# delldu/TransMVSNet

Measured on AMD Instinct MI355X. Metric: depth maps/sec @ DTU 864x1152 N=5 (48/32/8 hyp); Abs depth L1 vs ref, higher is better.
Workload: dtype f32; 1 GPU; DTU 864x1152, N=5 views, cascade 48/32/8, B=1, hot path from FeatureNet outputs (FMT+pathway+stage glue+cost volume+CostRegNet+softmax/WTA); global_batch=1, parallelism=replica1, launch=hip_graph replay

## Files before the change

### transmvsnet_amd/csrc/common.h

```cpp
#pragma once

#include <hip/hip_runtime.h>
#include <stdint.h>

#include "../../include/transmvs.h"

#define TMVS_CHECK_LAUNCH()                                   \
  do {                                                        \
    hipError_t _e = hipGetLastError();                        \
    if (_e != hipSuccess) return TMVS_ERR_HIP;                \
  } while (0)

namespace tmvs {

__device__ __forceinline__ float relu(float x) { return x > 0.f ? x : 0.f; }

typedef float floatx4_t __attribute__((ext_vector_type(4)));

struct LinAxis {
  int i0, i1;
  float l0, l1;
};
__device__ __forceinline__ LinAxis lin_axis(int dst, int in_size, int out_size) {
  const float scale = (float)in_size / (float)out_size;
  float src = scale * ((float)dst + 0.5f) - 0.5f;
  src = src < 0.f ? 0.f : src;
  LinAxis a;
  a.i0 = min((int)floorf(src), in_size - 1);
  a.i1 = a.i0 + (a.i0 < in_size - 1 ? 1 : 0);
  const float l = fminf(fmaxf(src - (float)a.i0, 0.f), 1.f);
  a.l1 = l;
  a.l0 = 1.f - l;
  return a;
}
__device__ __forceinline__ LinAxis lin_axis_x2(int dst, int in_size) {
  float src = 0.5f * ((float)dst + 0.5f) - 0.5f;
  src = src < 0.f ? 0.f : src;
  LinAxis a;
  a.i0 = (int)src;
  a.i0 = a.i0 < in_size - 1 ? a.i0 : in_size - 1;
  a.i1 = a.i0 + (a.i0 < in_size - 1 ? 1 : 0);
  a.l1 = src - (float)a.i0;
  a.l0 = 1.f - a.l1;
  return a;
}

__device__ __forceinline__ bool xcd_range_tap(int ntaps, int nblk, int& rb, int& k) {
  const int per = 8 * ntaps;
  const int grp = blockIdx.x / per, within = blockIdx.x % per;
  k = within / 8;
  rb = grp * 8 + within % 8;
  return rb < nblk;
}
static inline dim3 xcd_range_tap_grid(int ntaps, int nblk) { return dim3((unsigned)((nblk + 7) / 8 * 8 * ntaps)); }

__device__ __forceinline__ void chunk_row_coords(long v, int H, int W, int& b, int& y, int& x) {
  const long vl = v & ~63L;
  const unsigned lo = __builtin_amdgcn_readfirstlane((unsigned)vl);
  const unsigned hi = __builtin_amdgcn_readfirstlane((unsigned)((unsigned long)vl >> 32));
  const long vb = (long)(((unsigned long)hi << 32) | lo);
  const long t = vb / W;
  x = (int)(vb - t * W) + (int)(v - vb);
  y = (int)(t % H);
  b = (int)(t / H);
  while (x >= W) {
    x -= W;
    if (++y == H) {
      y = 0;
      ++b;
    }
  }
}

__device__ __forceinline__ void chunk_row_coords3(long v, int D, int H, int W, int& b, int& z, int& y, int& x) {
  const long vl = v & ~63L;
  const unsigned lo = __builtin_amdgcn_readfirstlane((unsigned)vl);
  const unsigned hi = __builtin_amdgcn_readfirstlane((unsigned)((unsigned long)vl >> 32));
  const long vb = (long)(((unsigned long)hi << 32) | lo);
  long t = vb / W;
  x = (int)(vb - t * W) + (int)(v - vb);
  y = (int)(t % H);
  t /= H;
  z = (int)(t % D);
  b = (int)(t / D);
  while (x >= W) {
    x -= W;
    if (++y == H) {
      y = 0;
      if (++z == D) {
        z = 0;
        ++b;
      }
    }
  }
}

// ... 85 lines not shown
```

### transmvsnet_amd/csrc/fmt.hip

```cpp
#include "fmt_common.h"

namespace tmvs {

__global__ __launch_bounds__(256) void fmt_embed_kernel(const float* __restrict__ feat, long view_stride,
                                                        const float* __restrict__ pe, int pe_h, int pe_w, int H, int W,
                                                        int nv, float* __restrict__ tokens) {
  __shared__ float tile[64][kD + 1];
  const int HW = H * W;
  const int p0 = blockIdx.x * 64;
  const int px = threadIdx.x & 63, c0 = threadIdx.x >> 6;
  const int p = p0 + px;
  const bool in = p < HW;
  const int y = in ? p / W : 0, x = in ? p - y * W : 0;
  float pv[kD / 4];
#pragma unroll
  for (int k = 0; k < kD / 4; ++k) pv[k] = in ? pe[((size_t)(c0 + 4 * k) * pe_h + y) * pe_w + x] : 0.f;
  const int tp = threadIdx.x >> 3, q = threadIdx.x & 7;
  float t[kD / 4];
  auto load = [&](int v) {
    const float* f = feat + (size_t)v * view_stride;
#pragma unroll
    for (int k = 0; k < kD / 4; ++k) t[k] = in ? f[(size_t)(c0 + 4 * k) * HW + p] : 0.f;
  };
  load(0);
#pragma unroll 1
  for (int v = 0; v < nv; ++v) {
    __syncthreads();
#pragma unroll
    for (int k = 0; k < kD / 4; ++k) tile[px][c0 + 4 * k] = t[k] + pv[k];
    __syncthreads();
    if (v + 1 < nv) load(v + 1);
#pragma unroll
    for (int h = 0; h < 2; ++h) {
      const int r = tp + 32 * h;
      if (p0 + r < HW)
        *reinterpret_cast<float4*>(tokens + ((size_t)v * HW + p0 + r) * kD + 4 * q) =
            make_float4(tile[r][4 * q], tile[r][4 * q + 1], tile[r][4 * q + 2], tile[r][4 * q + 3]);
    }
  }
}

__device__ __forceinline__ int kfeat(int s, int g) { return 16 * (s >> 2) + 4 * g + (s & 3); }

template <int OUT, int IN, bool TRANS>
__device__ __forceinline__ void stage_afrag(const float* __restrict__ W, float* __restrict__ lds) {
  constexpr int N = OUT * IN;
  for (int idx = threadIdx.x; idx < N; idx += blockDim.x) {
    const int j = idx & 3, l = (idx >> 2) & 63, rest = idx >> 8;
    const int s4 = rest % (IN / 16), mb = rest / (IN / 16);
    const int s = 4 * s4 + j;
    const int o = 16 * mb + (l & 15), i = kfeat(s, l >> 4);
    lds[idx] = TRANS ? W[i * OUT + o] : W[o * IN + i];
  }
}

template <int OUT, int IN>
__device__ __forceinline__ void mfma_linear_lds(const float* __restrict__ fl, const floatx4_t (&in)[IN / 16],
                                                floatx4_t (&acc)[OUT / 16], int lane) {
#pragma unroll
  for (int mb = 0; mb < OUT / 16; ++mb) acc[mb] = floatx4_t{0.f, 0.f, 0.f, 0.f};
#pragma unroll
  for (int s4 = 0; s4 < IN / 16; ++s4) {
    float4 a4[OUT / 16];
#pragma unroll
    for (int mb = 0; mb < OUT / 16; ++mb) a4[mb] = ld4(fl + ((mb * (IN / 16) + s4) * 64 + lane) * 4);
#pragma unroll
    for (int j = 0; j < 4; ++j)
#pragma unroll
      for (int mb = 0; mb < OUT / 16; ++mb)
        acc[mb] = __builtin_amdgcn_mfma_f32_16x16x4f32(j == 0 ? a4[mb].x : j == 1 ? a4[mb].y : j == 2 ? a4[mb].z : a4[mb].w,
                                                       in[s4][j], acc[mb], 0, 0, 0);
  }
}

__device__ __forceinline__ int wave_index() { return __builtin_amdgcn_readfirstlane(threadIdx.x >> 6); }
__device__ __forceinline__ int first_tile(int wv, int tpw) { return (blockIdx.x * 4 + wv) * tpw; }
__device__ __forceinline__ int opaque_zero() {
  int salt = 0;
  asm volatile("" : "+s"(salt));
  return salt;
}
template <typename T>
__device__ __forceinline__ T* row(T* base, int t, int n) { return base + (size_t)(t < n ? t : n - 1) * kD; }
__device__ __forceinline__ void ld4(const float* p, float (&a)[4]) {
  const float4 t = ld4(p);
  a[0] = t.x, a[1] = t.y, a[2] = t.z, a[3] = t.w;
}

__device__ __forceinline__ float token_sum(float v) {
  v += __shfl_xor(v, 16, 64);
  v += __shfl_xor(v, 32, 64);
  return v;
}

__device__ __forceinline__ void layer_norm_frag(floatx4_t (&x)[2], const float* __restrict__ g,
                                                const float* __restrict__ b, int lane) {
  float s = 0.f;
#pragma unroll
  for (int mb = 0; mb < 2; ++mb)
#pragma unroll
    for (int r = 0; r < 4; ++r) s += x[mb][r];
  const float mean = token_sum(s) / (float)kD;
  float v = 0.f;
#pragma unroll
  for (int mb = 0; mb < 2; ++mb)
#pragma unroll
    for (int r = 0; r < 4; ++r) {
      const float d = x[mb][r] - mean;
      v = fmaf(d, d, v);
    }
  const float rstd = 1.f / sqrtf(token_sum(v) / (float)kD + kLnEps);
  const float bias = -rstd * mean;
#pragma unroll
  for (int mb = 0; mb < 2; ++mb) {
    float gg[4], bb[4];
    ld4(g + 16 * mb + 4 * (lane >> 4), gg);
    ld4(b + 16 * mb + 4 * (lane >> 4), bb);
#pragma unroll
    for (int r = 0; r < 4; ++r) x[mb][r] = fmaf(fmaf(x[mb][r], rstd, bias), gg[r], bb[r]);
  }
}

__device__ __forceinline__ void load_token_frag(const float* __restrict__ row, floatx4_t (&x)[2], int lane) {
#pragma unroll
  for (int mb = 0; mb < 2; ++mb) {
    const float4 t = ld4(row + 16 * mb + 4 * (lane >> 4));
    x[mb] = floatx4_t{t.x, t.y, t.z, t.w};
  }
}

constexpr int kKvTilesPerWave = 8;

template <int OFF>
__device__ __forceinline__ float xor_add(float x) {
  return x + __int_as_float(xor_lane_dpp<OFF>(__float_as_int(x)));
}
__device__ __forceinline__ float xor_sum16(float x) { return xor_add<8>(xor_add<4>(xor_add<2>(xor_add<1>(x)))); }

__global__ __launch_bounds__(256) void fmt_kv_partial_kernel(const float* __restrict__ src, int S,
                                                              const float* __restrict__ w,
                                                              float* __restrict__ partial, int tpw) {
  __shared__ float red[4][kKV];
  __shared__ __attribute__((aligned(16))) float frag[2 * 32 * 32];
  const int v = blockIdx.y;
  const int lane = threadIdx.x & 63, wv = wave_index();
  const int g = lane >> 4;
  stage_afrag<32, 32, true>(w + TMVS_ENC_WK, frag);
  stage_afrag<32, 32, true>(w + TMVS_ENC_WV, frag + 1024);
  float bk[2][4], bv[2][4];
#pragma unroll
  for (int mb = 0; mb < 2; ++mb)
#pragma unroll
    for (int r = 0; r < 4; ++r) {
      bk[mb][r] = w[TMVS_ENC_BK + 16 * mb + 4 * g + r];
      bv[mb][r] = w[TMVS_ENC_BV + 16 * mb + 4 * g + r];
    }
  float kv[2][16], ks[2][4];
#pragma unroll
  for (int mb = 0; mb < 2; ++mb) {
// ... 2 lines not shown
#pragma unroll
    for (int i = 0; i < 4; ++i) ks[mb][i] = 0.f;
  }
  __syncthreads();
  const float* sv = src + (size_t)v * S * kD;
  const int tile0 = first_tile(wv, tpw);
  floatx4_t xa[2], xb[2];
  if (tile0 * 16 < S) load_token_frag(row(sv, tile0 * 16 + (lane & 15), S), xa, lane);
  auto tile = [&](int it, floatx4_t (&cur)[2], floatx4_t (&nxt)[2]) {
    const float* fr = frag + opaque_zero();
    const int t = (tile0 + it) * 16 + (lane & 15);
    const bool ok = t < S;
    const floatx4_t xin[2] = {cur[0], cur[1]};
    floatx4_t kk[2], vv[2];
    load_token_frag(row(sv, t + 16, S), nxt, lane);
    mfma_linear_lds<32, 32>(fr, xin, kk, lane);
    mfma_linear_lds<32, 32>(fr + 1024, xin, vv, lane);
#pragma unroll
    for (int mb = 0; mb < 2; ++mb) {
      float kh[4], vh[4];
#pragma unroll
      for (int r = 0; r < 4; ++r) {
        kh[r] = ok ? elu1(kk[mb][r] + bk[mb][r]) : 0.f;
        vh[r] = ok ? vv[mb][r] + bv[mb][r] : 0.f;
      }
#pragma unroll
      for (int m = 0; m < 4; ++m)
#pragma unroll
        for (int d = 0; d < 4; ++d) kv[mb][m * 4 + d] = fmaf(kh[d], vh[m], kv[mb][m * 4 + d]);
#pragma unroll
      for (int d = 0; d < 4; ++d) ks[mb][d] += kh[d];
    }
  };
#pragma unroll 1
  for (int it = 0; it < tpw; ++it) {
    if ((tile0 + it) * 16 >= S) break;
    tile(it, xa, xb);
    xa[0] = xb[0];
    xa[1] = xb[1];
  }
#pragma unroll
  for (int mb = 0; mb < 2; ++mb) {
#pragma unroll
    for (int i = 0; i < 16; ++i) kv[mb][i] = xor_sum16(kv[mb][i]);
#pragma unroll
    for (int i = 0; i < 4; ++i) ks[mb][i] = xor_sum16(ks[mb][i]);
  }
  if ((lane & 15) == 0) {
#pragma unroll
    for (int mb = 0; mb < 2; ++mb) {
      const int h = 4 * mb + g;
#pragma unroll
      for (int i = 0; i < 16; ++i) red[wv][kv_at(h, i >> 2, i & 3)] = kv[mb][i];
#pragma unroll
      for (int i = 0; i < 4; ++i) red[wv][ksum_at(h, i)] = ks[mb][i];
    }
  }
  __syncthreads();
  if (threadIdx.x < kKV) {
    const int i = threadIdx.x;
    partial[((size_t)v * gridDim.x + blockIdx.x) * kKV + i] = (red[0][i] + red[1][i]) + (red[2][i] + red[3][i]);
  }
}

__global__ __launch_bounds__(1024) void fmt_kv_combine_kernel(const float* __restrict__ partial, int nblk,
                                                              float* __restrict__ kv) {
  __shared__ float red[32][32];
  const int v = blockIdx.x;
  const int e = blockIdx.y * 32 + (threadIdx.x & 31);
  const int g = threadIdx.x >> 5;
  float s = 0.f;
#pragma unroll 4
  for (int b = g; b < nblk; b += 32) s += partial[((size_t)v * nblk + b) * kKV + e];
  red[g][threadIdx.x & 31] = s;
  __syncthreads();
  if (g == 0) {
    float t = red[0][threadIdx.x];
#pragma unroll
    for (int k = 1; k < 32; ++k) t += red[k][threadIdx.x];
    kv[(size_t)v * kKV + e] = t;
  }
}

__global__ __launch_bounds__(256) void fmt_apply_kernel(float* __restrict__ x, int L, const float* __restrict__ kvg,
                                                        long kv_stride, const float* __restrict__ w, int tpw) {
  __shared__ __attribute__((aligned(16))) float kvs[kKV];
  constexpr int kVB2 = 128, kVLN = 160;
  __shared__ __attribute__((aligned(16))) float vec[288];
  const int v = blockIdx.y;
  const int lane = threadIdx.x & 63, wv = wave_index();
  const int g = lane >> 4;
  if (threadIdx.x < kKV) kvs[threadIdx.x] = kvg[(size_t)v * kv_stride + threadIdx.x];
  for (int i = threadIdx.x; i < 288; i += blockDim.x)
    vec[i] = i < 32 ? w[TMVS_ENC_BQ + i] : i < 64 ? w[TMVS_ENC_BO + i - 32] : i < 128 ? w[TMVS_ENC_B1 + i - 64]
                                                                                      : w[TMVS_ENC_B2 + i - kVB2];
  __shared__ __attribute__((aligned(16))) float frag[32 * 32 * 2 + 64 * 32 * 2];
  stage_afrag<32, 32, false>(w + TMVS_ENC_WQ, frag);
  stage_afrag<32, 32, false>(w + TMVS_ENC_WO, frag + 1024);
  stage_afrag<64, 32, false>(w + TMVS_ENC_W1, frag + 2048);
  stage_afrag<32, 64, true>(w + TMVS_ENC_W2T, frag + 4096);
  __syncthreads();
  float* xv = x + (size_t)v * L * kD;
  const int tile0 = first_tile(wv, tpw);
  floatx4_t xa[2], xb[2];
  load_token_frag(row(xv, tile0 * 16 + (lane & 15), L), xa, lane);
  auto tile = [&](int it, floatx4_t (&cur)[2], floatx4_t (&nxt)[2]) {
    const int salt = opaque_zero();
    const float* fr = frag + salt;
    const float* vb = vec + salt;
    const int t = (tile0 + it) * 16 + (lane & 15);
    const bool ok = t < L;
    float* out = row(xv, t, L);
    floatx4_t xs[2] = {cur[0], cur[1]};
    load_token_frag(row(xv, t + 16, L), nxt, lane);
    floatx4_t q[2], msg[2];
    mfma_linear_lds<32, 32>(fr, xs, q, lane);
#pragma unroll
    for (int mb = 0; mb < 2; ++mb) {
      const int h = 4 * mb + g;
      float bq[4], ksum[4], kvm[4][4];
      ld4(vb + 4 * h, bq);
      ld4(kvs + ksum_at(h, 0), ksum);
#pragma unroll
      for (int m = 0; m < 4; ++m) ld4(kvs + kv_at(h, m, 0), kvm[m]);
      float qe[4];
#pragma unroll
      for (int d = 0; d < 4; ++d) qe[d] = elu1(q[mb][d] + bq[d]);
      float den = 0.f;
#pragma unroll
      for (int d = 0; d < 4; ++d) den = fmaf(qe[d], ksum[d], den);
      const float z = 1.f / (den + kAttnEps);
#pragma unroll
      for (int m = 0; m < 4; ++m) {
        float num = 0.f;
#pragma unroll
        for (int d = 0; d < 4; ++d) num = fmaf(qe[d], kvm[m][d], num);
        msg[mb][m] = num * z;
      }
    }
    floatx4_t a[2];
    mfma_linear_lds<32, 32>(fr + 1024, msg, a, lane);
#pragma unroll
    for (int mb = 0; mb < 2; ++mb) {
      float bo[4];
      ld4(vb + 32 + 16 * mb + 4 * g, bo);
#pragma unroll
      for (int r = 0; r < 4; ++r) xs[mb][r] = xs[mb][r] + (a[mb][r] + bo[r]);
    }
    layer_norm_frag(xs, vb + kVLN, vb + kVLN + kD, lane);
    floatx4_t hdn[4], ff[2];
    mfma_linear_lds<64, 32>(fr + 2048, xs, hdn, lane);
#pragma unroll
    for (int mb = 0; mb < 4; ++mb) {
      float b1[4];
      ld4(vb + 64 + 16 * mb + 4 * g, b1);
#pragma unroll
      for (int r = 0; r < 4; ++r) hdn[mb][r] = relu(hdn[mb][r] + b1[r]);
    }
    mfma_linear_lds<32, 64>(fr + 4096, hdn, ff, lane);
#pragma unroll
    for (int mb = 0; mb < 2; ++mb) {
      float b2[4];
      ld4(vb + kVB2 + 16 * mb + 4 * g, b2);
#pragma unroll
      for (int r = 0; r < 4; ++r) xs[mb][r] = xs[mb][r] + (ff[mb][r] + b2[r]);
    }
    layer_norm_frag(xs, vb + kVLN + 2 * kD, vb + kVLN + 3 * kD, lane);
    if (ok) {
#pragma unroll
      for (int mb = 0; mb < 2; ++mb)
        *reinterpret_cast<float4*>(out + 16 * mb + 4 * g) = make_float4(xs[mb][0], xs[mb][1], xs[mb][2], xs[mb][3]);
    }
  };
#pragma unroll 1
  for (int it = 0; it < tpw; it += 2) {
    if ((tile0 + it) * 16 >= L) break;
    tile(it, xa, xb);
    if (it + 1 >= tpw || (tile0 + it + 1) * 16 >= L) break;
    tile(it + 1, xb, xa);
  }
}

template <typename K>
static long block_slots(K kernel) {
  int dev = 0, cus = 0, per = 0;
  (void)hipGetDevice(&dev);
  (void)hipDeviceGetAttribute(&cus, hipDeviceAttributeMultiprocessorCount, dev);
  if (hipOccupancyMaxActiveBlocksPerMultiprocessor(&per, kernel, 256, 0) != hipSuccess || per <= 0) per = 4;
  return (long)(cus > 0 ? cus : 256) * per;
}
static int wave_slots_apply() {
  static long slots = 0;
  if (!slots) slots = 4 * block_slots(fmt_apply_kernel);
  return (int)slots;
}

static int kv_tiles_per_wave(int nv, int S) {
  const int tiles = (S + 15) / 16;
  int tpw = kKvTilesPerWave;
  while (tpw > 2 && (long)nv * ((tiles + tpw - 1) / tpw) < 2048) tpw >>= 1;
  return tpw;
}
static int kv_nblk(int nv, int S) {
  const int per = 16 * 4 * kv_tiles_per_wave(nv, S);
  return (S + per - 1) / per;
}
static int apply_tiles_per_wave(int nv, int L) {
  const long tiles = (long)nv * ((L + 15) / 16);
  return (int)std::max<long>(1, (tiles + wave_slots_apply() - 1) / wave_slots_apply());
}
static int apply_nblk(int L, int tpw) { return (L + 16 * 4 * tpw - 1) / (16 * 4 * tpw); }

}

using namespace tmvs;

extern "C" int tmvs_fmt_embed(const float* feat, long feat_view_stride, const float* pe, int pe_h, int pe_w, int nv,
                              int channels, int height, int width, float* tokens, void* stream) {
  if (!feat || !pe || !tokens || nv <= 0 || height <= 0 || width <= 0) return TMVS_ERR_ARG;
  if (channels != kD || height > pe_h || width > pe_w) return TMVS_ERR_SHAPE;
  const int HW = height * width;
  hipLaunchKernelGGL(fmt_embed_kernel, dim3((HW + 63) / 64), dim3(256), 0, (hipStream_t)stream, feat,
                     feat_view_stride, pe, pe_h, pe_w, height, width, nv, tokens);
  TMVS_CHECK_LAUNCH();
  return TMVS_OK;
}

extern "C" size_t tmvs_fmt_kv_grouped_workspace(int nv, int group_nv, int s_tokens) {
  if (nv <= 0 || group_nv <= 0 || s_tokens <= 0) return 0;
  return (size_t)nv * kv_nblk(group_nv, s_tokens) * kKV * sizeof(float);
}

extern "C" size_t tmvs_fmt_kv_workspace(int nv, int s_tokens) { return tmvs_fmt_kv_grouped_workspace(nv, nv, s_tokens); }

extern "C" int tmvs_fmt_kv_grouped(const float* source, int nv, int group_nv, int s_tokens, const float* enc_w,
                                   void* workspace, size_t workspace_bytes, float* kv, void* stream) {
  if (!source || !enc_w || !workspace || !kv || nv <= 0 || group_nv <= 0 || s_tokens <= 0) return TMVS_ERR_ARG;
  if (workspace_bytes < tmvs_fmt_kv_grouped_workspace(nv, group_nv, s_tokens)) return TMVS_ERR_ARG;
  const int nblk = kv_nblk(group_nv, s_tokens);
  hipStream_t st = (hipStream_t)stream;
  hipLaunchKernelGGL(fmt_kv_partial_kernel, dim3(nblk, nv), dim3(256), 0, st, source, s_tokens, enc_w,
                     (float*)workspace, kv_tiles_per_wave(group_nv, s_tokens));
  TMVS_CHECK_LAUNCH();
  hipLaunchKernelGGL(fmt_kv_combine_kernel, dim3(nv, kKV / 32), dim3(1024), 0, st, (const float*)workspace, nblk, kv);
  TMVS_CHECK_LAUNCH();
  return TMVS_OK;
}

extern "C" int tmvs_fmt_kv(const float* source, int nv, int s_tokens, const float* enc_w, void* workspace,
                           size_t workspace_bytes, float* kv, void* stream) {
  return tmvs_fmt_kv_grouped(source, nv, nv, s_tokens, enc_w, workspace, workspace_bytes, kv, stream);
}

extern "C" int tmvs_fmt_apply_tiled(float* x, int nv, int l_tokens, const float* kv, long kv_view_stride,
                                    const float* enc_w, int tiles_per_wave, void* stream) {
  if (!x || !kv || !enc_w || nv <= 0 || l_tokens <= 0 || kv_view_stride < 0) return TMVS_ERR_ARG;
  const int tpw = tiles_per_wave > 0 ? tiles_per_wave : apply_tiles_per_wave(nv, l_tokens);
  hipLaunchKernelGGL(fmt_apply_kernel, dim3(apply_nblk(l_tokens, tpw), nv), dim3(256), 0, (hipStream_t)stream, x,
                     l_tokens, kv, kv_view_stride, enc_w, tpw);
  TMVS_CHECK_LAUNCH();
  return TMVS_OK;
}

extern "C" int tmvs_fmt_apply(float* x, int nv, int l_tokens, const float* kv, long kv_view_stride,
                              const float* enc_w, void* stream) {
  return tmvs_fmt_apply_tiled(x, nv, l_tokens, kv, kv_view_stride, enc_w, 0, stream);
}
```

### transmvsnet_amd/csrc/pipeline.hip

```cpp
#include "common.h"

static size_t align_up256(size_t v) { return (v + 255) & ~(size_t)255; }
static size_t fmt_kv_slab(int nv, int l_tokens) {
  const size_t a = tmvs_fmt_kv_workspace(nv, l_tokens), b = tmvs_fmt_kv_workspace(1, l_tokens);
  return align_up256(a > b ? a : b);
}

extern "C" size_t tmvs_fmt_forward_workspace(int nv, int l_tokens) {
  return fmt_kv_slab(nv, l_tokens) + align_up256((size_t)(4 + nv) * TMVS_KV_NFLOATS * 4);
}

extern "C" int tmvs_fmt_forward(const float* stage1, long view_stride, const float* pe, int pe_h, int pe_w, int nv,
                                int height, int width, const float* const* enc_w, void* workspace,
                                size_t workspace_bytes, float* tokens, void* stream) {
  if (!stage1 || !pe || !enc_w || !workspace || !tokens || nv <= 0) return TMVS_ERR_ARG;
  for (int i = 0; i < 8; ++i)
    if (!enc_w[i]) return TMVS_ERR_ARG;
  const int L = height * width;
  if (workspace_bytes < tmvs_fmt_forward_workspace(nv, L)) return TMVS_ERR_ARG;
  char* ws = (char*)workspace;
  const size_t slab = fmt_kv_slab(nv, L);
  void* kv_ws = ws;
  float* kv_cross = (float*)(ws + slab);
  float* kv_self = kv_cross + 4 * TMVS_KV_NFLOATS;
  int rc;
  if ((rc = tmvs_fmt_embed(stage1, view_stride, pe, pe_h, pe_w, nv, 32, height, width, tokens, stream))) return rc;
  float* src = tokens + (size_t)L * 32;
  for (int j = 0; j < 4; ++j) {
    const int i = 2 * j;
    if ((rc = tmvs_fmt_kv(tokens, nv, L, enc_w[i], kv_ws, slab, kv_self, stream))) return rc;
    if ((rc = tmvs_fmt_apply(tokens, nv, L, kv_self, TMVS_KV_NFLOATS, enc_w[i], stream))) return rc;
    if (nv == 1) continue;
    if ((rc = tmvs_fmt_kv(tokens, 1, L, enc_w[i + 1], kv_ws, slab, kv_cross + j * TMVS_KV_NFLOATS, stream))) return rc;
    if ((rc = tmvs_fmt_apply(src, nv - 1, L, kv_cross + j * TMVS_KV_NFLOATS, 0, enc_w[i + 1], stream))) return rc;
  }
  return TMVS_OK;
}

static size_t fmt_split_slab_main(int nv, int l_tokens) {
  return align_up256(tmvs_fmt_kv_grouped_workspace(nv - 1, nv, l_tokens));
}
static size_t fmt_split_slab_side(int nv, int l_tokens) {
  const size_t a = tmvs_fmt_kv_grouped_workspace(1, nv, l_tokens), b = tmvs_fmt_kv_workspace(1, l_tokens);
  return align_up256(a > b ? a : b);
}

extern "C" size_t tmvs_fmt_forward_split_workspace(int nv, int l_tokens) {
  if (nv < 2) return tmvs_fmt_forward_workspace(nv, l_tokens);
  return fmt_split_slab_main(nv, l_tokens) + fmt_split_slab_side(nv, l_tokens) +
         align_up256((size_t)(4 + 1 + (nv - 1)) * TMVS_KV_NFLOATS * 4);
}

namespace {
constexpr int kSplitRefTilesPerWave = 2;


struct SplitEvents {
  hipEvent_t ev[6];
  bool ok;
};
SplitEvents* split_events() {
  constexpr int kMaxDev = 16;
  thread_local SplitEvents cache[kMaxDev] = {};
  int dev = 0;
  if (hipGetDevice(&dev) != hipSuccess || dev < 0 || dev >= kMaxDev) return nullptr;
  SplitEvents& e = cache[dev];
  if (!e.ok) {
    for (int i = 0; i < 6; ++i)
      if (hipEventCreateWithFlags(&e.ev[i], hipEventDisableTiming) != hipSuccess) return nullptr;
    e.ok = true;
  }
  return &e;
}
}

extern "C" int tmvs_fmt_forward_split(const float* stage1, long view_stride, const float* pe, int pe_h, int pe_w,
                                      int nv, int height, int width, const float* const* enc_w, void* workspace,
                                      size_t workspace_bytes, float* tokens, void* stream, void* side_stream) {
  if (!side_stream || nv < 2 || side_stream == stream)
    return tmvs_fmt_forward(stage1, view_stride, pe, pe_h, pe_w, nv, height, width, enc_w, workspace, workspace_bytes,
                            tokens, stream);
  if (!stage1 || !pe || !enc_w || !workspace || !tokens) return TMVS_ERR_ARG;
  for (int i = 0; i < 8; ++i)
    if (!enc_w[i]) return TMVS_ERR_ARG;
  const int L = height * width;
  if (workspace_bytes < tmvs_fmt_forward_split_workspace(nv, L)) return TMVS_ERR_ARG;
  SplitEvents* e = split_events();
  if (!e) return TMVS_ERR_HIP;
  hipStream_t ms = (hipStream_t)stream, ss = (hipStream_t)side_stream;
  char* ws = (char*)workspace;
  const size_t sm = fmt_split_slab_main(nv, L), sd = fmt_split_slab_side(nv, L);
  void* slab_main = ws;
  void* slab_side = ws + sm;
  float* kv_cross = (float*)(ws + sm + sd);
  float* kv_ref = kv_cross + 4 * TMVS_KV_NFLOATS;
  float* kv_src = kv_ref + TMVS_KV_NFLOATS;
  int rc;
  if ((rc = tmvs_fmt_embed(stage1, view_stride, pe, pe_h, pe_w, nv, 32, height, width, tokens, stream))) return rc;
  if (hipEventRecord(e->ev[0], ms) != hipSuccess || hipStreamWaitEvent(ss, e->ev[0], 0) != hipSuccess)
    return TMVS_ERR_HIP;
  float* src = tokens + (size_t)L * 32;
  auto ref_layer = [&](int j) -> int {
    const int i = 2 * j;
    int r;
    if ((r = tmvs_fmt_kv_grouped(tokens, 1, nv, L, enc_w[i], slab_side, sd, kv_ref, ss))) return r;
    if ((r = tmvs_fmt_apply_tiled(tokens, 1, L, kv_ref, TMVS_KV_NFLOATS, enc_w[i], kSplitRefTilesPerWave, ss))) return r;
    if ((r = tmvs_fmt_kv(tokens, 1, L, enc_w[i + 1], slab_side, sd, kv_cross + j * TMVS_KV_NFLOATS, ss))) return r;
    return hipEventRecord(e->ev[1 + j], ss) != hipSuccess ? TMVS_ERR_HIP : TMVS_OK;
  };
  auto src_self = [&](int j) -> int {
    const int i = 2 * j;
    int r;
    if ((r = tmvs_fmt_kv_grouped(src, nv - 1, nv, L, enc_w[i], slab_main, sm, kv_src, ms))) return r;
    return tmvs_fmt_apply(src, nv - 1, L, kv_src, TMVS_KV_NFLOATS, enc_w[i], ms);
  };
  auto src_cross = [&](int j) -> int {
    if (hipStreamWaitEvent(ms, e->ev[1 + j], 0) != hipSuccess) return TMVS_ERR_HIP;
    return tmvs_fmt_apply(src, nv - 1, L, kv_cross + j * TMVS_KV_NFLOATS, 0, enc_w[2 * j + 1], ms);
  };
  for (int j = 0; j < 4; ++j)
    if ((rc = ref_layer(j))) return rc;
  for (int j = 0; j < 4; ++j)
    if ((rc = src_self(j)) || (rc = src_cross(j))) return rc;
  if (hipEventRecord(e->ev[5], ss) != hipSuccess) return TMVS_ERR_HIP;
  if (hipStreamWaitEvent(ms, e->ev[5], 0) != hipSuccess) return TMVS_ERR_HIP;
  return TMVS_OK;
}

extern "C" size_t tmvs_depth_stage_workspace(int ndepth, int height, int width, int base_ch) {
  const size_t vol = (size_t)ndepth * height * width * 4;
  return align_up256(vol) + align_up256(tmvs_costregnet_workspace(1, ndepth, height, width, base_ch));
}

extern "C" int tmvs_depth_stage(const float* depth_values, int n_values, const float* prev_depth, int prev_h,
                                int prev_w, const float* feat, int n_views, int channels, int ndepth, float ratio,
                                int full_h, int full_w, int stage_scale, const float* proj, const float* pw_params,
                                float* view_w, int vw_shift, int warp_flags, const TmvsCostRegWeights* cr, void* workspace,
                                size_t workspace_bytes, float clamp_lo, float clamp_hi, float* hyp_out,
                                float* prob_out, float* depth_out, float* depth_raw_out, float* conf_out,
                                void* stream) {
  if (!feat || !view_w || !cr || !workspace || !hyp_out || n_views < 2) return TMVS_ERR_ARG;
  const int h = full_h / stage_scale, w = full_w / stage_scale;
  if (workspace_bytes < tmvs_depth_stage_workspace(ndepth, h, w, cr->base_ch)) return TMVS_ERR_ARG;
  const size_t vol = (size_t)ndepth * h * w;
  char* ws = (char*)workspace;
  float* sim = (float*)ws;
  char* crws = ws + align_up256(vol * 4);
  const size_t crbytes = workspace_bytes - align_up256(vol * 4);
  const int V = n_views - 1;
  int rc;
  if ((rc = tmvs_stage_hypotheses(depth_values, n_values, prev_depth, prev_h, prev_w, 1, ndepth, ratio, full_h, full_w,
                                  stage_scale, hyp_out, stream)))
    return rc;
  const float* ref = feat;
  const float* src = feat + (size_t)h * w * channels;
  if (pw_params)
    rc = tmvs_warp_corr(ref, src, proj, hyp_out, nullptr, 0, 0, V, pw_params, 1, V, channels, ndepth, h, w,
                        warp_flags & TMVS_WARP_ROT_PLAIN, sim,
                        nullptr, view_w, stream);
  else
    rc = tmvs_warp_corr(ref, src, proj, hyp_out, view_w, vw_shift, 0, V, nullptr, 1, V, channels, ndepth, h, w,
                        warp_flags & TMVS_WARP_ROT_PLAIN, sim, nullptr, nullptr, stream);
  if (rc) return rc;
  return tmvs_costregnet_wta(sim, hyp_out, 1, ndepth, h, w, cr, crws, crbytes, clamp_lo, clamp_hi, prob_out, depth_out,
                             depth_raw_out, conf_out, stream);
}
```

### transmvsnet_amd/ops.py

```python
from __future__ import annotations

import ctypes
import functools

import numpy as np
import torch

from . import _lib

_lib_h = _lib.load


_TIMER = None


def set_timer(timer):
    global _TIMER
    _TIMER = timer


def _call(name, *args, span=None):
    fn = getattr(_lib_h(), name)
    args = [a.data_ptr() if isinstance(a, torch.Tensor) else a for a in args]
    tok = _TIMER.begin(span or name) if _TIMER is not None else None
# ... 219 lines not shown

def _layer_tensor(op, name, t, device):
    if t is None:
        return
    if not t.is_cuda or t.device != device:
        raise ValueError(f"{op}: {name} must be a GPU tensor on x's device (the HIP path has no CPU fallback)")
    if t.dtype != torch.float32 or not t.is_contiguous():
        raise ValueError(f"{op}: {name} must be contiguous float32")


def _layer_like(op, name, t, shape, device):
    _layer_tensor(op, name, t, device)
    if t is not None and tuple(t.shape) != tuple(shape):
        raise ValueError(f"{op}: {name} must be a contiguous {list(shape)} tensor, not {list(t.shape)}")


def _layer_no_alias(op, skip, out):
    if skip is not None and out is not None and skip.data_ptr() == out.data_ptr():
        raise ValueError(f"{op}: out must not alias skip (the kernels read skip while they write out)")


def _conv_out_dhw(d, h, w, stride):
    return (d, h, w) if stride == 1 else ((d - 1) // 2 + 1, (h - 1) // 2 + 1, (w - 1) // 2 + 1)


@_on_tensor_device
def conv3d_bn_relu(x, wpk, alpha, shift, cout, stride, out=None):
    _layer_args("conv3d_bn_relu", x, wpk, alpha, shift, cout)
    b, d, h, w, cin = x.shape
    shape = (b, *_conv_out_dhw(d, h, w, stride), cout)
    _layer_like("conv3d_bn_relu", "out", out, shape, x.device)
    y = torch.empty(shape, device=x.device) if out is None else out
    _launch("tmvs_conv3d_bn_relu", x, b, cin, d, h, w, wpk, alpha, shift, cout, stride, y)
    return y


@_on_tensor_device
def deconv3d_bn_relu_add(x, wpk, alpha, shift, cout, skip, out=None, route=None, max_workgroups=0):
    _layer_args("deconv3d_bn_relu_add", x, wpk, alpha, shift, cout)
    b, d, h, w, cin = x.shape
    shape = (b, 2 * d, 2 * h, 2 * w, cout)
    if skip is None:
        raise ValueError("deconv3d_bn_relu_add: skip is required")
    _layer_like("deconv3d_bn_relu_add", "skip", skip, shape, x.device)
    _layer_like("deconv3d_bn_relu_add", "out", out, shape, x.device)
    _layer_no_alias("deconv3d_bn_relu_add", skip, out)
    y = torch.empty(shape, device=x.device) if out is None else out
    if route not in (None, "generic", "persistent"):
        raise ValueError(f"deconv3d_bn_relu_add: unknown route {route!r}")
    bound = (int(max_workgroups),) if route == "persistent" else ()
    _launch("tmvs_deconv3d_bn_relu_add" + ("_" + route if route else ""), x, b, cin, d, h, w, wpk, alpha, shift, cout,
            skip, y, *bound)
    return y


@_on_tensor_device
def fmt_embed(feat_nchw, pe, out_tokens):
    nv, c, h, w = feat_nchw.shape
    _launch("tmvs_fmt_embed", feat_nchw, c * h * w, pe, pe.shape[1], pe.shape[2], nv, c, h, w, out_tokens)
    return out_tokens


@_on_tensor_device
def fmt_kv(source_tokens, enc_w, out=None, group_nv=None):
    nv, s, _ = source_tokens.shape
    group_nv = nv if group_nv is None else int(group_nv)
    nbytes = _lib_h().tmvs_fmt_kv_grouped_workspace(nv, group_nv, s)
    ws = torch.empty(max(1, nbytes // 4), device=source_tokens.device)
    kv = out if out is not None else torch.empty(nv, _lib.KV_NFLOATS, device=source_tokens.device)
    _launch("tmvs_fmt_kv_grouped", source_tokens, nv, group_nv, s, enc_w, ws, ws.numel() * 4, kv, span="tmvs_fmt_kv")
    return kv


@_on_tensor_device
def fmt_apply(x_tokens, kv, enc_w, shared_kv=False, tiles_per_wave=0):
    nv, l, _ = x_tokens.shape
    _launch("tmvs_fmt_apply_tiled", x_tokens, nv, l, kv, 0 if shared_kv else _lib.KV_NFLOATS, enc_w,
            int(tiles_per_wave), span="tmvs_fmt_apply")
    return x_tokens


@_on_tensor_device
def fmt_pathway(coarse_nhwc, lateral_nchw, w_reduce, w_smooth, out=None):
    nv, h, w, cc = coarse_nhwc.shape
    cf = lateral_nchw.shape[1]
    if out is None:
        out = torch.empty(nv, 2 * h, 2 * w, cf, device=coarse_nhwc.device)
    elif tuple(out.shape) != (nv, 2 * h, 2 * w, cf) or not out.is_contiguous():
        raise ValueError(f"fmt_pathway: out must be a contiguous [{nv},{2 * h},{2 * w},{cf}] tensor")
    _launch("tmvs_fmt_pathway", coarse_nhwc, lateral_nchw, cf * 4 * h * w, w_reduce, w_smooth, nv, cc, cf, h, w, out)
    return out


@_on_tensor_device
def fmt_forward(stage1_nchw, pe, enc_list, tokens=None, side_stream=None):
    _dev(stage1_nchw, "stage1")
    nv, c, h, w = stage1_nchw.shape
    tokens = torch.empty(nv, h * w, c, device=stage1_nchw.device) if tokens is None else tokens
    name = "tmvs_fmt_forward_split" if side_stream is not None and nv > 1 else "tmvs_fmt_forward"
    ws, nbytes = _workspace(name + "_workspace", nv, h * w, device=stage1_nchw.device)
    ptrs = (ctypes.c_void_p * 8)(*[e.data_ptr() for e in enc_list])
    args = (stage1_nchw, c * h * w, pe, pe.shape[1], pe.shape[2], nv, h, w, ptrs, ws, nbytes, tokens)
    if name == "tmvs_fmt_forward":
        _launch(name, *args)
    else:
        _call(name, *args, _stream(), side_stream.cuda_stream, span="tmvs_fmt_forward")
        if not torch.cuda.is_current_stream_capturing():
            ws.record_stream(side_stream)
            tokens.record_stream(side_stream)
    return tokens


@_on_tensor_device
def depth_stage(depth_values, prev_depth, feat_nhwc, ndepth, ratio, full_hw, stage_scale, proj12, pw_params,
                view_w, vw_shift, cr_weights, clamp=(425.0, 935.0), rot_order="auto"):
    _dev(depth_values, "depth_values")
    _dev(prev_depth, "prev_depth")
    _dev(feat_nhwc, "feat")
    _dev(view_w, "view_w")
    n, h, w, c = feat_nhwc.shape
    dev = feat_nhwc.device
    hyp = torch.empty(1, ndepth, h, w, device=dev)
    prob = torch.empty_like(hyp)
    depth = torch.empty(1, h, w, device=dev)
    raw = torch.empty_like(depth)
    conf = torch.empty_like(depth)
    proj = np.ascontiguousarray(proj12, np.float32).reshape(n - 1, 12)
    pw = None if pw_params is None else np.ascontiguousarray(pw_params, np.float32)
    ph, pwd = (prev_depth.shape[-2], prev_depth.shape[-1]) if prev_depth is not None else (0, 0)
    _launch("tmvs_depth_stage", depth_values, depth_values.shape[-1], prev_depth, ph, pwd, feat_nhwc, n, c, ndepth,
            ratio, full_hw[0], full_hw[1], stage_scale, proj.ctypes.data, None if pw is None else pw.ctypes.data,
            view_w, vw_shift, warp_flags(rot_order, h * w), ctypes.byref(cr_weights),
            *_workspace("tmvs_depth_stage_workspace", ndepth, h, w, cr_weights.base_ch, device=dev), clamp[0], clamp[1],
            hyp, prob, depth, raw, conf)
    return {"depth": depth, "photo_confidence": conf, "prob_volume": prob, "depth_values": hyp}, raw


def deform_conv2d_pack(weight):
    w = np.ascontiguousarray(weight.detach().float().cpu().numpy(), np.float32)
    co, ci = w.shape[:2]
    out = np.empty(_lib_h().tmvs_deform_conv2d_packed_floats(co), np.float32)
    _lib.check(_lib_h().tmvs_deform_conv2d_pack(w.ctypes.data, co, ci, out.ctypes.data), "tmvs_deform_conv2d_pack")
    return torch.from_numpy(out)


@_on_tensor_device
def deform_conv2d(x_nhwc, offset_mask, w_packed, bias, cout, bn=None, relu=False, want_nhwc=False):
    for t, n in ((x_nhwc, "x_nhwc"), (offset_mask, "offset_mask"), (w_packed, "w_packed"), (bias, "bias")):
        _dev(t, n)
    b, h, w, cin = x_nhwc.shape
    if offset_mask.shape != (b, 27, h, w) or not offset_mask.is_contiguous() or not x_nhwc.is_contiguous():
        raise ValueError("deform_conv2d: expects contiguous x_nhwc [B,H,W,C] and offset_mask [B,27,H,W]")
    out = torch.empty(b, cout, h, w, device=x_nhwc.device)
    out_nhwc = torch.empty(b, h, w, cout, device=x_nhwc.device) if want_nhwc else None
    alpha, shift = bn if bn is not None else (None, None)
    _launch("tmvs_deform_conv2d", x_nhwc, offset_mask, w_packed, bias, alpha, shift, int(relu), b, cin, cout, h, w, out,
            out_nhwc)
    return (out, out_nhwc) if want_nhwc else out


@_on_tensor_device
def dcn_fused(x_nhwc, wom_packed, bom, w_packed, bias, cout, bn=None, relu=False, want_nchw=True, want_nhwc=False):
    for t, n in ((x_nhwc, "x_nhwc"), (wom_packed, "wom_packed"), (bom, "bom"), (w_packed, "w_packed"), (bias, "bias")):
        _dev(t, n)
    if not (want_nchw or want_nhwc):
        raise ValueError("dcn_fused: request at least one output layout")
# ... 844 lines not shown
```

Before: 304.3 depth_maps/s.

## Fuse source self and cross FMT attention layers into one paired apply kernel

Source views now run their self-attention apply and the following cross-attention apply in a single kernel launch. The token fragments stay in registers between the two layers, which removes a global write and re-read of the tokens and one launch per layer pair. The fused kernel uses 8-wave blocks and stages both layers' weights in LDS, which raises LDS use per block and may reduce occupancy. Weight staging into the MFMA fragment layout also switches to vectorised float4 loads. The ops.py change only adds device checks on the pathway tensors.

```diff
diff --git a/transmvsnet_amd/csrc/common.h b/transmvsnet_amd/csrc/common.h
--- a/transmvsnet_amd/csrc/common.h
+++ b/transmvsnet_amd/csrc/common.h
@@ -12,6 +12,9 @@
   } while (0)
 
 namespace tmvs {
+
+int fmt_apply_pair(float* x, int nv, int l_tokens, const float* kv0, const float* enc_w0, const float* kv1,
+                   const float* enc_w1, void* stream);
 
 __device__ __forceinline__ float relu(float x) { return x > 0.f ? x : 0.f; }
 
diff --git a/transmvsnet_amd/csrc/fmt.hip b/transmvsnet_amd/csrc/fmt.hip
--- a/transmvsnet_amd/csrc/fmt.hip
+++ b/transmvsnet_amd/csrc/fmt.hip
@@ -40,17 +40,19 @@
   }
 }
 
-__device__ __forceinline__ int kfeat(int s, int g) { return 16 * (s >> 2) + 4 * g + (s & 3); }
-
 template <int OUT, int IN, bool TRANS>
 __device__ __forceinline__ void stage_afrag(const float* __restrict__ W, float* __restrict__ lds) {
   constexpr int N = OUT * IN;
-  for (int idx = threadIdx.x; idx < N; idx += blockDim.x) {
-    const int j = idx & 3, l = (idx >> 2) & 63, rest = idx >> 8;
-    const int s4 = rest % (IN / 16), mb = rest / (IN / 16);
-    const int s = 4 * s4 + j;
-    const int o = 16 * mb + (l & 15), i = kfeat(s, l >> 4);
-    lds[idx] = TRANS ? W[i * OUT + o] : W[o * IN + i];
+  const bool aligned = (reinterpret_cast<size_t>(W) & 15) == 0;
+  for (int e = 4 * threadIdx.x; e < N; e += 4 * blockDim.x) {
+    const float4 t = aligned ? ld4(W + e) : make_float4(W[e], W[e + 1], W[e + 2], W[e + 3]);
+    const int o = TRANS ? e % OUT : e / IN, i = TRANS ? e / OUT : e % IN;
+    const int at = (((o >> 4) * (IN / 16) + (i >> 4)) * 64 + 16 * ((i >> 2) & 3) + (o & 15)) * 4 + (i & 3);
+    if (TRANS) {
+      lds[at] = t.x, lds[at + 4] = t.y, lds[at + 8] = t.z, lds[at + 12] = t.w;
+    } else {
+      *reinterpret_cast<float4*>(lds + at) = t;
+    }
   }
 }
 
@@ -74,7 +76,8 @@
 }
 
 __device__ __forceinline__ int wave_index() { return __builtin_amdgcn_readfirstlane(threadIdx.x >> 6); }
-__device__ __forceinline__ int first_tile(int wv, int tpw) { return (blockIdx.x * 4 + wv) * tpw; }
+template <int WPB = 4>
+__device__ __forceinline__ int first_tile(int wv, int tpw) { return (blockIdx.x * WPB + wv) * tpw; }
 __device__ __forceinline__ int opaque_zero() {
   int salt = 0;
   asm volatile("" : "+s"(salt));
@@ -243,90 +246,110 @@
   }
 }
 
-__global__ __launch_bounds__(256) void fmt_apply_kernel(float* __restrict__ x, int L, const float* __restrict__ kvg,
-                                                        long kv_stride, const float* __restrict__ w, int tpw) {
-  __shared__ __attribute__((aligned(16))) float kvs[kKV];
-  constexpr int kVB2 = 128, kVLN = 160;
-  __shared__ __attribute__((aligned(16))) float vec[288];
-  const int v = blockIdx.y;
-  const int lane = threadIdx.x & 63, wv = wave_index();
-  const int g = lane >> 4;
-  if (threadIdx.x < kKV) kvs[threadIdx.x] = kvg[(size_t)v * kv_stride + threadIdx.x];
-  for (int i = threadIdx.x; i < 288; i += blockDim.x)
+constexpr int kVB2 = 128, kVLN = 160, kVec = 288;
+constexpr int kApplyFrag = 32 * 32 * 2 + 64 * 32 * 2;
+__device__ __forceinline__ void stage_layer(const float* __restrict__ w, const float* __restrict__ kv,
+                                            float* __restrict__ kvs, float* __restrict__ vec,
+                                            float* __restrict__ frag) {
+  if (threadIdx.x < kKV) kvs[threadIdx.x] = kv[threadIdx.x];
+  for (int i = threadIdx.x; i < kVec; i += blockDim.x)
     vec[i] = i < 32 ? w[TMVS_ENC_BQ + i] : i < 64 ? w[TMVS_ENC_BO + i - 32] : i < 128 ? w[TMVS_ENC_B1 + i - 64]
                                                                                       : w[TMVS_ENC_B2 + i - kVB2];
-  __shared__ __attribute__((aligned(16))) float frag[32 * 32 * 2 + 64 * 32 * 2];
   stage_afrag<32, 32, false>(w + TMVS_ENC_WQ, frag);
   stage_afrag<32, 32, false>(w + TMVS_ENC_WO, frag + 1024);
   stage_afrag<64, 32, false>(w + TMVS_ENC_W1, frag + 2048);
   stage_afrag<32, 64, true>(w + TMVS_ENC_W2T, frag + 4096);
+}
+
+__device__ __forceinline__ void apply_layer(floatx4_t (&xs)[2], const float* fr, const float* vb, const float* kvs,
+                                            int lane) {
+  const int g = lane >> 4;
+  floatx4_t q[2], msg[2];
+  mfma_linear_lds<32, 32>(fr, xs, q, lane);
+#pragma unroll
+  for (int mb = 0; mb < 2; ++mb) {
+    const int h = 4 * mb + g;
+    float bq[4], ksum[4], kvm[4][4];
+    ld4(vb + 4 * h, bq);
+    ld4(kvs + ksum_at(h, 0), ksum);
+#pragma unroll
+    for (int m = 0; m < 4; ++m) ld4(kvs + kv_at(h, m, 0), kvm[m]);
+    float qe[4];
+#pragma unroll
+    for (int d = 0; d < 4; ++d) qe[d] = elu1(q[mb][d] + bq[d]);
+    float den = 0.f;
+#pragma unroll
+    for (int d = 0; d < 4; ++d) den = fmaf(qe[d], ksum[d], den);
+    const float z = 1.f / (den + kAttnEps);
+#pragma unroll
+    for (int m = 0; m < 4; ++m) {
+      float num = 0.f;
+#pragma unroll
+      for (int d = 0; d < 4; ++d) num = fmaf(qe[d], kvm[m][d], num);
+      msg[mb][m] = num * z;
+    }
+  }
+  floatx4_t a[2];
+  mfma_linear_lds<32, 32>(fr + 1024, msg, a, lane);
+#pragma unroll
+  for (int mb = 0; mb < 2; ++mb) {
+    float bo[4];
+    ld4(vb + 32 + 16 * mb + 4 * g, bo);
+#pragma unroll
+    for (int r = 0; r < 4; ++r) xs[mb][r] = xs[mb][r] + (a[mb][r] + bo[r]);
+  }
+  layer_norm_frag(xs, vb + kVLN, vb + kVLN + kD, lane);
+  floatx4_t hdn[4], ff[2];
+  mfma_linear_lds<64, 32>(fr + 2048, xs, hdn, lane);
+#pragma unroll
+  for (int mb = 0; mb < 4; ++mb) {
+    float b1[4];
+    ld4(vb + 64 + 16 * mb + 4 * g, b1);
+#pragma unroll
+    for (int r = 0; r < 4; ++r) hdn[mb][r] = relu(hdn[mb][r] + b1[r]);
+  }
+  mfma_linear_lds<32, 64>(fr + 4096, hdn, ff, lane);
+#pragma unroll
+  for (int mb = 0; mb < 2; ++mb) {
+    float b2[4];
+    ld4(vb + kVB2 + 16 * mb + 4 * g, b2);
+#pragma unroll
+    for (int r = 0; r < 4; ++r) xs[mb][r] = xs[mb][r] + (ff[mb][r] + b2[r]);
+  }
+  layer_norm_frag(xs, vb + kVLN + 2 * kD, vb + kVLN + 3 * kD, lane);
+}
+
+struct LayerArgs {
+  const float* w;
+  const float* kv;
+  long kv_stride;
+};
+template <int NL, int WPB>
+__device__ __forceinline__ void apply_tiles(float* __restrict__ x, int L, const LayerArgs (&layer)[NL], int tpw) {
+  __shared__ __attribute__((aligned(16))) float kvs[NL][kKV];
+  __shared__ __attribute__((aligned(16))) float vec[NL][kVec];
+  __shared__ __attribute__((aligned(16))) float frag[NL][kApplyFrag];
+  const int v = blockIdx.y;
+  const int lane = threadIdx.x & 63, wv = wave_index();
+  const int g = lane >> 4;
+#pragma unroll
+  for (int i = 0; i < NL; ++i)
+    stage_layer(layer[i].w, layer[i].kv + (size_t)v * layer[i].kv_stride, kvs[i], vec[i], frag[i]);
   __syncthreads();
   float* xv = x + (size_t)v * L * kD;
-  const int tile0 = first_tile(wv, tpw);
+  const int tile0 = first_tile<WPB>(wv, tpw);
   floatx4_t xa[2], xb[2];
   load_token_frag(row(xv, tile0 * 16 + (lane & 15), L), xa, lane);
   auto tile = [&](int it, floatx4_t (&cur)[2], floatx4_t (&nxt)[2]) {
     const int salt = opaque_zero();
-    const float* fr = frag + salt;
-    const float* vb = vec + salt;
     const int t = (tile0 + it) * 16 + (lane & 15);
     const bool ok = t < L;
     float* out = row(xv, t, L);
     floatx4_t xs[2] = {cur[0], cur[1]};
     load_token_frag(row(xv, t + 16, L), nxt, lane);
-    floatx4_t q[2], msg[2];
-    mfma_linear_lds<32, 32>(fr, xs, q, lane);
-#pragma unroll
-    for (int mb = 0; mb < 2; ++mb) {
-      const int h = 4 * mb + g;
-      float bq[4], ksum[4], kvm[4][4];
-      ld4(vb + 4 * h, bq);
-      ld4(kvs + ksum_at(h, 0), ksum);
-#pragma unroll
-      for (int m = 0; m < 4; ++m) ld4(kvs + kv_at(h, m, 0), kvm[m]);
-      float qe[4];
-#pragma unroll
-      for (int d = 0; d < 4; ++d) qe[d] = elu1(q[mb][d] + bq[d]);
-      float den = 0.f;
-#pragma unroll
-      for (int d = 0; d < 4; ++d) den = fmaf(qe[d], ksum[d], den);
-      const float z = 1.f / (den + kAttnEps);
-#pragma unroll
-      for (int m = 0; m < 4; ++m) {
-        float num = 0.f;
-#pragma unroll
-        for (int d = 0; d < 4; ++d) num = fmaf(qe[d], kvm[m][d], num);
-        msg[mb][m] = num * z;
-      }
-    }
-    floatx4_t a[2];
-    mfma_linear_lds<32, 32>(fr + 1024, msg, a, lane);
-#pragma unroll
-    for (int mb = 0; mb < 2; ++mb) {
-      float bo[4];
-      ld4(vb + 32 + 16 * mb + 4 * g, bo);
-#pragma unroll
-      for (int r = 0; r < 4; ++r) xs[mb][r] = xs[mb][r] + (a[mb][r] + bo[r]);
-    }
-    layer_norm_frag(xs, vb + kVLN, vb + kVLN + kD, lane);
-    floatx4_t hdn[4], ff[2];
-    mfma_linear_lds<64, 32>(fr + 2048, xs, hdn, lane);
-#pragma unroll
-    for (int mb = 0; mb < 4; ++mb) {
-      float b1[4];
-      ld4(vb + 64 + 16 * mb + 4 * g, b1);
-#pragma unroll
-      for (int r = 0; r < 4; ++r) hdn[mb][r] = relu(hdn[mb][r] + b1[r]);
-    }
-    mfma_linear_lds<32, 64>(fr + 4096, hdn, ff, lane);
-#pragma unroll
-    for (int mb = 0; mb < 2; ++mb) {
-      float b2[4];
-      ld4(vb + kVB2 + 16 * mb + 4 * g, b2);
-#pragma unroll
-      for (int r = 0; r < 4; ++r) xs[mb][r] = xs[mb][r] + (ff[mb][r] + b2[r]);
-    }
-    layer_norm_frag(xs, vb + kVLN + 2 * kD, vb + kVLN + 3 * kD, lane);
+    static_assert(NL == 1 || NL == 2, "layers per launch");
+    apply_layer(xs, frag[0] + salt, vec[0] + salt, kvs[0], lane);
+    if constexpr (NL == 2) apply_layer(xs, frag[1] + salt, vec[1] + salt, kvs[1], lane);
     if (ok) {
 #pragma unroll
       for (int mb = 0; mb < 2; ++mb)
@@ -342,17 +365,39 @@
   }
 }
 
+__global__ __launch_bounds__(256) void fmt_apply_kernel(float* __restrict__ x, int L, const float* __restrict__ kvg,
+                                                        long kv_stride, const float* __restrict__ w, int tpw) {
+  const LayerArgs layer[1] = {{w, kvg, kv_stride}};
+  apply_tiles<1, 4>(x, L, layer, tpw);
+}
+
+constexpr int kPairWaves = 8;
+__global__ __launch_bounds__(64 * kPairWaves) __attribute__((amdgpu_waves_per_eu(4))) void fmt_pair_kernel(float* __restrict__ x, int L,
+                                                                   const float* __restrict__ kv0, long kv0_stride,
+                                                                   const float* __restrict__ w0,
+                                                                   const float* __restrict__ kv1, long kv1_stride,
+                                                                   const float* __restrict__ w1, int tpw) {
+  const LayerArgs layer[2] = {{w0, kv0, kv0_stride}, {w1, kv1, kv1_stride}};
+  apply_tiles<2, kPairWaves>(x, L, layer, tpw);
+}
+
 template <typename K>
-static long block_slots(K kernel) {
+static long block_slots(K kernel, int threads = 256) {
   int dev = 0, cus = 0, per = 0;
   (void)hipGetDevice(&dev);
   (void)hipDeviceGetAttribute(&cus, hipDeviceAttributeMultiprocessorCount, dev);
-  if (hipOccupancyMaxActiveBlocksPerMultiprocessor(&per, kernel, 256, 0) != hipSuccess || per <= 0) per = 4;
+  if (hipOccupancyMaxActiveBlocksPerMultiprocessor(&per, kernel, threads, 0) != hipSuccess || per <= 0)
+    per = 1024 / threads;
   return (long)(cus > 0 ? cus : 256) * per;
 }
 static int wave_slots_apply() {
   static long slots = 0;
   if (!slots) slots = 4 * block_slots(fmt_apply_kernel);
+  return (int)slots;
+}
+static int wave_slots_pair() {
+  static long slots = 0;
+  if (!slots) slots = kPairWaves * block_slots(fmt_pair_kernel, 64 * kPairWaves);
   return (int)slots;
 }
 
@@ -366,11 +411,11 @@
   const int per = 16 * 4 * kv_tiles_per_wave(nv, S);
   return (S + per - 1) / per;
 }
-static int apply_tiles_per_wave(int nv, int L) {
+static int apply_tiles_per_wave(int nv, int L, int wave_slots) {
   const long tiles = (long)nv * ((L + 15) / 16);
-  return (int)std::max<long>(1, (tiles + wave_slots_apply() - 1) / wave_slots_apply());
-}
-static int apply_nblk(int L, int tpw) { return (L + 16 * 4 * tpw - 1) / (16 * 4 * tpw); }
+  return (int)std::max<long>(1, (tiles + wave_slots - 1) / wave_slots);
+}
+static int apply_nblk(int L, int tpw, int wpb) { return (L + 16 * wpb * tpw - 1) / (16 * wpb * tpw); }
 
 }
 
@@ -416,8 +461,8 @@
 extern "C" int tmvs_fmt_apply_tiled(float* x, int nv, int l_tokens, const float* kv, long kv_view_stride,
                                     const float* enc_w, int tiles_per_wave, void* stream) {
   if (!x || !kv || !enc_w || nv <= 0 || l_tokens <= 0 || kv_view_stride < 0) return TMVS_ERR_ARG;
-  const int tpw = tiles_per_wave > 0 ? tiles_per_wave : apply_tiles_per_wave(nv, l_tokens);
-  hipLaunchKernelGGL(fmt_apply_kernel, dim3(apply_nblk(l_tokens, tpw), nv), dim3(256), 0, (hipStream_t)stream, x,
+  const int tpw = tiles_per_wave > 0 ? tiles_per_wave : apply_tiles_per_wave(nv, l_tokens, wave_slots_apply());
+  hipLaunchKernelGGL(fmt_apply_kernel, dim3(apply_nblk(l_tokens, tpw, 4), nv), dim3(256), 0, (hipStream_t)stream, x,
                      l_tokens, kv, kv_view_stride, enc_w, tpw);
   TMVS_CHECK_LAUNCH();
   return TMVS_OK;
@@ -427,3 +472,13 @@
                               const float* enc_w, void* stream) {
   return tmvs_fmt_apply_tiled(x, nv, l_tokens, kv, kv_view_stride, enc_w, 0, stream);
 }
+
+int tmvs::fmt_apply_pair(float* x, int nv, int l_tokens, const float* kv0, const float* enc_w0, const float* kv1,
+                         const float* enc_w1, void* stream) {
+  if (!x || !kv0 || !enc_w0 || !kv1 || !enc_w1 || nv <= 0 || l_tokens <= 0) return TMVS_ERR_ARG;
+  const int tpw = apply_tiles_per_wave(nv, l_tokens, wave_slots_pair());
+  hipLaunchKernelGGL(fmt_pair_kernel, dim3(apply_nblk(l_tokens, tpw, kPairWaves), nv), dim3(64 * kPairWaves), 0,
+                     (hipStream_t)stream, x, l_tokens, kv0, (long)kKV, enc_w0, kv1, 0L, enc_w1, tpw);
+  TMVS_CHECK_LAUNCH();
+  return TMVS_OK;
+}
diff --git a/transmvsnet_amd/csrc/pipeline.hip b/transmvsnet_amd/csrc/pipeline.hip
--- a/transmvsnet_amd/csrc/pipeline.hip
+++ b/transmvsnet_amd/csrc/pipeline.hip
@@ -29,10 +29,12 @@
   for (int j = 0; j < 4; ++j) {
     const int i = 2 * j;
     if ((rc = tmvs_fmt_kv(tokens, nv, L, enc_w[i], kv_ws, slab, kv_self, stream))) return rc;
-    if ((rc = tmvs_fmt_apply(tokens, nv, L, kv_self, TMVS_KV_NFLOATS, enc_w[i], stream))) return rc;
+    if ((rc = tmvs_fmt_apply(tokens, 1, L, kv_self, TMVS_KV_NFLOATS, enc_w[i], stream))) return rc;
     if (nv == 1) continue;
     if ((rc = tmvs_fmt_kv(tokens, 1, L, enc_w[i + 1], kv_ws, slab, kv_cross + j * TMVS_KV_NFLOATS, stream))) return rc;
-    if ((rc = tmvs_fmt_apply(src, nv - 1, L, kv_cross + j * TMVS_KV_NFLOATS, 0, enc_w[i + 1], stream))) return rc;
+    if ((rc = tmvs::fmt_apply_pair(src, nv - 1, L, kv_self + TMVS_KV_NFLOATS, enc_w[i], kv_cross + j * TMVS_KV_NFLOATS,
+                                   enc_w[i + 1], stream)))
+      return rc;
   }
   return TMVS_OK;
 }
@@ -108,20 +110,17 @@
     if ((r = tmvs_fmt_kv(tokens, 1, L, enc_w[i + 1], slab_side, sd, kv_cross + j * TMVS_KV_NFLOATS, ss))) return r;
     return hipEventRecord(e->ev[1 + j], ss) != hipSuccess ? TMVS_ERR_HIP : TMVS_OK;
   };
-  auto src_self = [&](int j) -> int {
+  auto src_pair = [&](int j) -> int {
     const int i = 2 * j;
     int r;
     if ((r = tmvs_fmt_kv_grouped(src, nv - 1, nv, L, enc_w[i], slab_main, sm, kv_src, ms))) return r;
-    return tmvs_fmt_apply(src, nv - 1, L, kv_src, TMVS_KV_NFLOATS, enc_w[i], ms);
-  };
-  auto src_cross = [&](int j) -> int {
     if (hipStreamWaitEvent(ms, e->ev[1 + j], 0) != hipSuccess) return TMVS_ERR_HIP;
-    return tmvs_fmt_apply(src, nv - 1, L, kv_cross + j * TMVS_KV_NFLOATS, 0, enc_w[2 * j + 1], ms);
+    return tmvs::fmt_apply_pair(src, nv - 1, L, kv_src, enc_w[i], kv_cross + j * TMVS_KV_NFLOATS, enc_w[i + 1], ms);
   };
   for (int j = 0; j < 4; ++j)
     if ((rc = ref_layer(j))) return rc;
   for (int j = 0; j < 4; ++j)
-    if ((rc = src_self(j)) || (rc = src_cross(j))) return rc;
+    if ((rc = src_pair(j))) return rc;
   if (hipEventRecord(e->ev[5], ss) != hipSuccess) return TMVS_ERR_HIP;
   if (hipStreamWaitEvent(ms, e->ev[5], 0) != hipSuccess) return TMVS_ERR_HIP;
   return TMVS_OK;
diff --git a/transmvsnet_amd/ops.py b/transmvsnet_amd/ops.py
--- a/transmvsnet_amd/ops.py
+++ b/transmvsnet_amd/ops.py
@@ -325,6 +325,9 @@
 
 @_on_tensor_device
 def fmt_pathway(coarse_nhwc, lateral_nchw, w_reduce, w_smooth, out=None):
+    for name, t in (("coarse", coarse_nhwc), ("lateral", lateral_nchw), ("w_reduce", w_reduce), ("w_smooth", w_smooth),
+                    ("out", out)):
+        _dev(t, name)
     nv, h, w, cc = coarse_nhwc.shape
     cf = lateral_nchw.shape[1]
     if out is None:
```

Measured after the change: 308.3 depth_maps/s (median of 6 runs). 1.3% higher.
